# Westlake-AI/SemiReward

Hardware: AMD Instinct MI355X
Metric: unlabeled images/sec/node (FlexMatch+SR, ViT-S CIFAR-100) (higher is better)
Workload: dtype bf16

## Files before the change

### semireward_amd/csrc/attn_block.hip

```cpp
#include <stdlib.h>

#include <type_traits>
#include <utility>

#include "../../include/srhip.h"
#include "common.h"

namespace {

constexpr int HD = 64;
constexpr int DM = 384;
constexpr int NH = DM / HD;
constexpr int KS = DM / 32;
constexpr int SK = 64;
constexpr int ST_EL = 64 * SK;
constexpr int NS = 8;
constexpr int GS = 2;
constexpr int NG = NS / GS;
constexpr int SPM = DM / SK;
constexpr int SPH = 3 * SPM;
constexpr int NSTG = NH * SPH;
constexpr float LOG2E = 1.4426950408889634f;

typedef __attribute__((address_space(3))) void lds_void;
template <int N_>
__device__ __forceinline__ void wait_vm() { asm volatile("s_waitcnt vmcnt(%0)" ::"n"(N_) : "memory"); }
__device__ __forceinline__ void lds_barrier() {
  asm volatile("s_waitcnt lgkmcnt(0)" ::: "memory");
  __builtin_amdgcn_s_barrier();
  asm volatile("" ::: "memory");
}

__device__ __forceinline__ int fresh_lane() {
  int l;
  asm volatile("v_mbcnt_lo_u32_b32 %0, -1, 0\n\tv_mbcnt_hi_u32_b32 %0, -1, %0" : "=v"(l));
  return l;
}

__device__ __forceinline__ float max3_raw(float a, float b, float c) {
  return __builtin_amdgcn_fmed3f(__builtin_amdgcn_fmed3f(a, b, INFINITY), c, INFINITY);
}
__device__ __forceinline__ float rows_max(float x) {
  const unsigned u = __float_as_uint(x);
  const auto a = __builtin_amdgcn_permlane16_swap(u, u, false, false);
  const unsigned v = __float_as_uint(__builtin_amdgcn_fmed3f(__uint_as_float(a[0]), __uint_as_float(a[1]), INFINITY));
  const auto b = __builtin_amdgcn_permlane32_swap(v, v, false, false);
  return __builtin_amdgcn_fmed3f(__uint_as_float(b[0]), __uint_as_float(b[1]), INFINITY);
}
__device__ __forceinline__ float rows_sum(float x) {
  const unsigned u = __float_as_uint(x);
  const auto a = __builtin_amdgcn_permlane16_swap(u, u, false, false);
  const unsigned v = __float_as_uint(__uint_as_float(a[0]) + __uint_as_float(a[1]));
  const auto b = __builtin_amdgcn_permlane32_swap(v, v, false, false);
  return __uint_as_float(b[0]) + __uint_as_float(b[1]);
}

__device__ __forceinline__ f32x4_t mfma16(u32x4_t a, u32x4_t b, f32x4_t c) {
  return __builtin_amdgcn_mfma_f32_16x16x32_bf16(__builtin_bit_cast(bf16x8_t, a), __builtin_bit_cast(bf16x8_t, b), c, 0, 0, 0);
}
__device__ __forceinline__ u32x4_t ldf(const bf16_t* p) { return *reinterpret_cast<const u32x4_t*>(p); }
__device__ __forceinline__ u32x4_t pack8v(f32x4_t lo, f32x4_t hi) {
  return u32x4_t{pack_bf2(lo[0], lo[1]), pack_bf2(lo[2], lo[3]), pack_bf2(hi[0], hi[1]), pack_bf2(hi[2], hi[3])};
}
constexpr int vt_pitch(int NP) { return ((NP / 2) % 64 == 16 || (NP / 2) % 64 == 48) ? NP : NP + 32; }
__device__ __forceinline__ int swz4(int row) { return (0x78 >> (((row >> 2) & 3) * 2)) & 3; }
constexpr int nkt_of(int N) { return 2 * ((N + 31) / 32); }

template <class F, int... Is>
__device__ __forceinline__ void static_for_impl(F&& f, std::integer_sequence<int, Is...>) { (f(std::integral_constant<int, Is>{}), ...); }
template <int N, class F>
__device__ __forceinline__ void static_for(F&& f) { static_for_impl(f, std::make_integer_sequence<int, N>{}); }

struct AbArgs {
  const bf16_t* xnb;
  const bf16_t* qx;
  const float* bqkv;
  const bf16_t* W;
  bf16_t* out;
  const float* osc;
  float scale;
  int B;
};

template <int N, int DBG>
__global__ __launch_bounds__(512, 2) void attn_block_kernel(AbArgs a) {
  constexpr int NKT = nkt_of(N), NP = NKT * 16, TP = vt_pitch(NP);
  constexpr int NQT = (N + 15) / 16;
  constexpr bool EXTRA = NQT == 17;
  static_assert(NQT <= 16 || (EXTRA && N == 257), "two token tiles per wave (+ one extra token)");
  constexpr int NKT_LO = (N - 1) / 16;
  extern __shared__ __attribute__((aligned(16))) bf16_t sm[];
  bf16_t* ring = sm;
  bf16_t* Ks = ring + NS * ST_EL;
  bf16_t* Vt = Ks + NP * HD;
  bf16_t* sx = Vt + HD * TP;
  float* sbias = reinterpret_cast<float*>(sx + 3 * DM);
  const int tid = threadIdx.x, lane = tid & 63;
  const int wave = __builtin_amdgcn_readfirstlane(tid >> 6);
  const int l15 = lane & 15, g = lane >> 4;
  const int img = blockIdx.x;
  const float osc = a.osc ? a.osc[img] : 1.0f;
  const int hpw = NH / gridDim.y, hbeg = blockIdx.y * hpw, hend = hbeg + hpw;
  const size_t row0 = (size_t)img * N;

  const int rho = 8 * wave + (lane >> 3);
  const int srcc = (lane & 7) ^ ((rho >> 1) & 7);
  const int fperm = (rho & 32) + 8 * ((rho & 15) >> 2) + 4 * ((rho >> 4) & 1) + (rho & 3);
  const int vo_kq = (fperm * DM + srcc * 8) * 2, vo_v = (rho * DM + srcc * 8) * 2;
  const __amdgpu_buffer_rsrc_t rw = __builtin_amdgcn_make_buffer_rsrc(const_cast<bf16_t*>(a.W), 0, 3 * DM * DM * 2, 0x00020000);
  constexpr int OOB = 0x7ffffff0;
  auto issue = [&](auto rc, int h) __attribute__((always_inline)) {
    constexpr int r0 = decltype(rc)::value, r = r0 % SPH, m = r / SPM, kc = r % SPM;
    const int hh = h + r0 / SPH;
    const bool valid = hh < hend;
    constexpr int brow = m == 0 ? DM : m == 1 ? 2 * DM : 0;
    lds_void* dst = (lds_void*)(ring + (r0 % NS >= 0 ? ((hh * SPH + r) & (NS - 1)) : 0) * ST_EL + wave * 8 * SK);
    if constexpr ((DBG & 4) != 0) return;
    __builtin_amdgcn_raw_ptr_buffer_load_lds(rw, dst, 16, valid ? (m == 1 ? vo_v : vo_kq) : OOB,
                                             valid ? ((brow + hh * HD) * DM + kc * SK) * 2 : 0, 0, 0);
  };
  issue(std::integral_constant<int, 0>{}, hbeg); issue(std::integral_constant<int, 1>{}, hbeg);
  issue(std::integral_constant<int, 2>{}, hbeg); issue(std::integral_constant<int, 3>{}, hbeg);
  static_assert((NG - 2) * GS == 4, "prologue issues the first two groups");

  for (int i = tid; i < 3 * DM; i += 512) sbias[i] = a.bqkv[i];
  if (EXTRA && tid < 3 * DM / 8) reinterpret_cast<u32x4_t*>(sx)[tid] = ldf(a.qx + (size_t)img * 3 * DM + 8 * tid);
  for (int i = tid; i < (NP - N) * HD / 8; i += 512) reinterpret_cast<u32x4_t*>(Ks + N * HD)[i] = u32x4_t{0u, 0u, 0u, 0u};
  for (int i = tid; i < HD * TP / 8; i += 512) reinterpret_cast<u32x4_t*>(Vt)[i] = u32x4_t{0u, 0u, 0u, 0u};
  __syncthreads();

  u32x4_t xn[2][KS];
#pragma unroll
  for (int tt = 0; tt < 2; ++tt) {
    const bool have = tt == 0 || NQT - (EXTRA ? 1 : 0) == 16 || wave + 8 < NQT - (EXTRA ? 1 : 0);
    const int tok = min(16 * (wave + 8 * tt) + l15, N - 1);
    const bf16_t* xr = a.xnb + (row0 + tok) * DM + 8 * g;
#pragma unroll
    for (int k = 0; k < KS; ++k) xn[tt][k] = have ? ldf(xr + 32 * k) : u32x4_t{0u, 0u, 0u, 0u};
  }

  const int kc_ = g ^ ((l15 >> 1) & 7);
  const int fo0 = l15 * SK + (kc_ << 3), fo1 = l15 * SK + ((kc_ ^ 4) << 3);
  const int kof0 = l15 * HD + (kc_ << 3), kof1 = l15 * HD + ((kc_ ^ 4) << 3);
  const int vof = l15 * TP + ((g ^ swz4(l15)) << 3);
  const float sc2 = a.scale * LOG2E;

  auto sync_group = [&](auto rc, int h) __attribute__((always_inline)) {
    constexpr int r = decltype(rc)::value;
    if constexpr ((DBG & 4) == 0) wait_vm<GS*(NG - 3)>();
    __builtin_amdgcn_s_barrier();
    if constexpr ((DBG & 32) == 0) {
      issue(std::integral_constant<int, r + (NG - 2) * GS>{}, h);
      issue(std::integral_constant<int, r + (NG - 2) * GS + 1>{}, h);
    }
    static_assert(GS == 2, "two stages per group");
  };
  constexpr bool ALL2 = NQT - (EXTRA ? 1 : 0) == 16;
  const bool tile1 = ALL2 || wave + 8 < NQT - (EXTRA ? 1 : 0);

  u32x4_t qf[2][2];
  auto project = [&](auto mc, int h) __attribute__((always_inline)) {
    constexpr int M = decltype(mc)::value;
    f32x4_t acc[2][4];
    const float* bb = sbias + (M == 0 ? DM : M == 1 ? 2 * DM : 0) + h * HD;
#pragma unroll
    for (int t = 0; t < 4; ++t) {
      f32x4_t b4;
      if constexpr (M == 1) { const float b = bb[16 * t + l15]; b4 = f32x4_t{b, b, b, b}; }
      else b4 = *reinterpret_cast<const f32x4_t*>(bb + 32 * (t >> 1) + 8 * g + 4 * (t & 1));
      acc[0][t] = b4; acc[1][t] = b4;
    }
    u32x4_t fa[2][2];
    auto rd = [&](auto uc) __attribute__((always_inline)) {
      constexpr int u = decltype(uc)::value, j = u >> 1, hf = u & 1, stg = j >> 1, sh = j & 1;
      const bf16_t* tile = ring + ((h * SPH + M * SPM + stg) & (NS - 1)) * ST_EL;
      fa[u & 1][0] = ldf(tile + (2 * hf) * 16 * SK + (sh ? fo1 : fo0));
      fa[u & 1][1] = ldf(tile + (2 * hf + 1) * 16 * SK + (sh ? fo1 : fo0));
    };
    auto mm = [&](auto uc) __attribute__((always_inline)) {
      constexpr int u = decltype(uc)::value, j = u >> 1, hf = u & 1;
      u32x4_t(&fr)[2] = fa[u & 1];
      if constexpr ((DBG & 2) != 0) {
        asm volatile("" ::"v"(fr[0]), "v"(fr[1]));
      } else if constexpr (M != 1) {
#pragma unroll
        for (int t = 0; t < 2; ++t) {
          acc[0][2 * hf + t] = mfma16(fr[t], xn[0][j], acc[0][2 * hf + t]);
          acc[1][2 * hf + t] = mfma16(fr[t], xn[1][j], acc[1][2 * hf + t]);
        }
      } else {
#pragma unroll
        for (int t = 0; t < 2; ++t) {
          acc[0][2 * hf + t] = mfma16(xn[0][j], fr[t], acc[0][2 * hf + t]);
          acc[1][2 * hf + t] = mfma16(xn[1][j], fr[t], acc[1][2 * hf + t]);
        }
      }
    };
    sync_group(std::integral_constant<int, M * SPM>{}, h);
    rd(std::integral_constant<int, 0>{});
    static_for<2 * KS>([&](auto uc) __attribute__((always_inline)) {
      constexpr int u = decltype(uc)::value;
      if constexpr (u + 1 < 2 * KS) {
        if constexpr ((u + 1) % (4 * GS) == 0) sync_group(std::integral_constant<int, M * SPM + (u + 1) / 4>{}, h);
        rd(std::integral_constant<int, u + 1>{});
      }
      __builtin_amdgcn_sched_barrier(0);
      mm(uc);
      __builtin_amdgcn_sched_barrier(0);
      if constexpr ((DBG & 32) != 0 && u % 4 == 0) issue(std::integral_constant<int, M * SPM + u / 4 + (NG - 2) * GS>{}, h);
    });
    if constexpr (M == 0) {
      const int lnk = fresh_lane(), l15k = lnk & 15, gk = lnk >> 4;
#pragma unroll
      for (int tt = 0; tt < 2; ++tt) {
        if (tt == 1 && !tile1) break;
        const int key = 16 * (wave + 8 * tt) + l15k;
#pragma unroll
        for (int blk = 0; blk < 2; ++blk)
          *reinterpret_cast<u32x4_t*>(Ks + key * HD + (((4 * blk + gk) ^ ((key >> 1) & 7)) << 3)) = pack8v(acc[tt][2 * blk], acc[tt][2 * blk + 1]);
      }
      if (EXTRA && wave == 0) {
        const int ln_ = fresh_lane();
        if (ln_ < 8) *reinterpret_cast<u32x4_t*>(Ks + 256 * HD + (ln_ << 3)) = ldf(sx + DM + h * HD + 8 * ln_);
      }
    } else if constexpr (M == 1) {
      const int lnv = fresh_lane(), l15v = lnv & 15, gv = lnv >> 4;
#pragma unroll
      for (int tt = 0; tt < 2; ++tt) {
        if (tt == 1 && !tile1) break;
        const int T = wave + 8 * tt, u = T >> 1, e = T & 1;
#pragma unroll
        for (int t = 0; t < 4; ++t) {
          const int d = 16 * t + l15v;
          *reinterpret_cast<u32x2_t*>(Vt + d * TP + 32 * u + ((gv ^ swz4(d)) << 3) + 4 * e) =
              u32x2_t{pack_bf2(acc[tt][t][0], acc[tt][t][1]), pack_bf2(acc[tt][t][2], acc[tt][t][3])};
        }
      }
      if (EXTRA && wave == 1) {
        const int ln_ = fresh_lane();
        Vt[ln_ * TP + 256 + (swz4(ln_) << 3)] = sx[2 * DM + h * HD + ln_];
      }
    } else {
#pragma unroll
      for (int tt = 0; tt < 2; ++tt) {
        qf[tt][0] = pack8v(acc[tt][0], acc[tt][1]);
        qf[tt][1] = pack8v(acc[tt][2], acc[tt][3]);
      }
    }
  };
  using C0 = std::integral_constant<int, 0>;
  using C1 = std::integral_constant<int, 1>;
  using C2 = std::integral_constant<int, 2>;

#pragma unroll 1
  for (int h = hbeg; h < hend; ++h) {
    project(C0{}, h);
    project(C1{}, h);
    project(C2{}, h);
    lds_barrier();

    const int nq = (DBG & 1) ? 0 : (tile1 ? 2 : 1) + ((EXTRA && (DBG & 8) == 0 && (h & 7) == wave) ? 1 : 0);
#pragma unroll 1
    for (int qi = 0; qi < nq; ++qi) {
      const bool ext = EXTRA && qi == (tile1 ? 2 : 1);
      int qtok;
      if (ext) { qf[0][0] = ldf(sx + h * HD + 8 * g); qf[0][1] = ldf(sx + h * HD + 32 + 8 * g); qtok = 256 + l15; }
      else qtok = 16 * (wave + 8 * qi) + l15;
      const u32x4_t q0 = qf[0][0], q1 = qf[0][1];
      constexpr int CHT = 4, NCH = (NKT + CHT - 1) / CHT;
      f32x4_t o[4];
#pragma unroll
      for (int dt = 0; dt < 4; ++dt) o[dt] = f32x4_t{0.f, 0.f, 0.f, 0.f};
      float mrun = -INFINITY;
      f32x2_t psum = {0.f, 0.f};
      static_for<NCH>([&](auto cc) __attribute__((always_inline)) {
        constexpr int ch = decltype(cc)::value, t0 = ch * CHT, nt = (NKT - t0 < CHT) ? NKT - t0 : CHT;
        static_assert(nt % 2 == 0, "the PV product consumes key-tile pairs");
        f32x4_t s[nt];
        float mx = -INFINITY;
#pragma unroll
        for (int i = 0; i < nt; ++i) {
          const int t = t0 + i;
          const int nvalid = N - 16 * t;
          if (nvalid <= 0) continue;
          f32x4_t c = {0.f, 0.f, 0.f, 0.f};
          c = mfma16(ldf(Ks + t * 16 * HD + kof0), q0, c);
          c = mfma16(ldf(Ks + t * 16 * HD + kof1), q1, c);
          if (nvalid >= 16) {
            mx = max3_raw(mx, c[0], c[1]);
            mx = max3_raw(mx, c[2], c[3]);
          } else {
#pragma unroll
            for (int r = 0; r < 4; ++r) {
              if (r < nvalid) { c[r] = (4 * g + r < nvalid) ? c[r] : -INFINITY; mx = max3_raw(mx, c[r], c[r]); }
            }
          }
          s[i] = c;
          if ((i & 1) == 1) __builtin_amdgcn_sched_barrier(0);
        }
        mx = rows_max(mx);
        const float mnew = max3_raw(mrun, mx, mx);
        const float nmx = -mnew * sc2;
        if constexpr (ch > 0) {
          const float corr = fast_exp2(fmaf(mrun, sc2, nmx));
          psum *= corr;
#pragma unroll
          for (int dt = 0; dt < 4; ++dt) o[dt] *= corr;
        }
        mrun = mnew;
        const f32x4_t sc4 = {sc2, sc2, sc2, sc2}, nm4 = {nmx, nmx, nmx, nmx};
#pragma unroll
        for (int i = 0; i < nt; ++i) {
          const int nvalid = N - 16 * (t0 + i);
          if (nvalid >= 16) {
            const f32x4_t e = __builtin_elementwise_fma(s[i], sc4, nm4);
            const f32x4_t p = (DBG & 16) ? e : f32x4_t{fast_exp2(e[0]), fast_exp2(e[1]), fast_exp2(e[2]), fast_exp2(e[3])};
            s[i] = p;
            psum += f32x2_t{p[0], p[1]};
            psum += f32x2_t{p[2], p[3]};
          } else {
            f32x4_t p = {0.f, 0.f, 0.f, 0.f};
#pragma unroll
            for (int r = 0; r < 4; ++r)
              if (r < nvalid) { p[r] = fast_exp2(fmaf(s[i][r], sc2, nmx)); psum[r & 1] += p[r]; }
            s[i] = p;
          }
        }
#pragma unroll
        for (int u = 0; u < nt / 2; ++u) {
          const u32x4_t pb = pack8v(s[2 * u], s[2 * u + 1]);
#pragma unroll
          for (int dt = 0; dt < 4; ++dt) o[dt] = mfma16(ldf(Vt + dt * 16 * TP + 32 * (t0 / 2 + u) + vof), pb, o[dt]);
          __builtin_amdgcn_sched_barrier(0);
        }
      });
      float sum = psum[0] + psum[1];
      sum = rows_sum(sum);
      if (qtok < N && (!ext || l15 == 0)) {
        const float inv = osc / sum;
        bf16_t* op = a.out + (row0 + qtok) * DM + h * HD + g * 4;
#pragma unroll
        for (int dt = 0; dt < 4; ++dt) {
          uint2 v = {pack_bf2(o[dt][0] * inv, o[dt][1] * inv), pack_bf2(o[dt][2] * inv, o[dt][3] * inv)};
          *reinterpret_cast<uint2*>(op + dt * 16) = v;
        }
      }
      qf[0][0] = qf[1][0]; qf[0][1] = qf[1][1];
    }
  }
}

template <int N, int DBG = 0>
int launch(const AbArgs& a, hipStream_t s) {
  constexpr int NKT = nkt_of(N), NP = NKT * 16, TP = vt_pitch(NP);
  const size_t smem = (size_t)(NS * ST_EL + NP * HD + HD * TP + 3 * DM) * sizeof(bf16_t) + (size_t)(3 * DM) * sizeof(float);
  auto kern = attn_block_kernel<N, DBG>;
  (void)hipFuncSetAttribute((const void*)kern, hipFuncAttributeMaxDynamicSharedMemorySize, (int)smem);
  int split = 1;
  for (int c : {2, 3, 6}) if (a.B * c <= 256) split = c;
  if (const char* e = SR_TUNE_ENV("SRHIP_AB_SPLIT")) { const int v = atoi(e); if (v == 1 || v == 2 || v == 3 || v == 6) split = v; }
  SR_LAUNCH(kern, dim3(a.B, split), dim3(512), smem, s, a);
  SR_CHECK_LAUNCH();
  return SR_OK;
}

}

extern "C" int srhip_attn_block_supported(int N, int D, int H) { return (D == DM && H == NH && (N == 257 || N == 197)) ? 1 : 0; }

extern "C" int srhip_attn_block_fused(const void* xn_bf16, const void* Wqkv, const float* bqkv, const void* qkv_extra, void* out,
                                      const float* out_scale, int B, int N, int D, int H, float scale, void* stream) {
  if (!xn_bf16 || !Wqkv || !bqkv || !out || B <= 0) return SR_EINVAL;
  if (!srhip_attn_block_supported(N, D, H)) return SR_EINVAL;
  if (N == 257 && !qkv_extra) return SR_EINVAL;
  if (((uintptr_t)xn_bf16 | (uintptr_t)Wqkv | (uintptr_t)out | (uintptr_t)bqkv | (uintptr_t)qkv_extra) & 15) return SR_EINVAL;
  AbArgs a;
  a.xnb = (const bf16_t*)xn_bf16; a.qx = (const bf16_t*)qkv_extra; a.bqkv = bqkv; a.W = (const bf16_t*)Wqkv; a.out = (bf16_t*)out;
  a.scale = scale; a.B = B; a.osc = out_scale;
  hipStream_t s = (hipStream_t)stream;
#ifdef SRHIP_TUNING
  switch (SR_TUNE_ENV("SRHIP_AB_DEBUG") ? atoi(SR_TUNE_ENV("SRHIP_AB_DEBUG")) : 0) {
    case 1: return N == 257 ? launch<257, 1>(a, s) : launch<197, 1>(a, s);
    case 2: return N == 257 ? launch<257, 2>(a, s) : launch<197, 2>(a, s);
    case 3: return N == 257 ? launch<257, 3>(a, s) : launch<197, 3>(a, s);
    case 4: return N == 257 ? launch<257, 4>(a, s) : launch<197, 4>(a, s);
    case 6: return N == 257 ? launch<257, 6>(a, s) : launch<197, 6>(a, s);
    case 7: return N == 257 ? launch<257, 7>(a, s) : launch<197, 7>(a, s);
    case 8: return N == 257 ? launch<257, 8>(a, s) : launch<197, 8>(a, s);
    case 16: return N == 257 ? launch<257, 16>(a, s) : launch<197, 16>(a, s);
    default: break;
  }
#endif
  static const int spread = SR_TUNE_ENV("SRHIP_ATTN_SPREAD") ? atoi(SR_TUNE_ENV("SRHIP_ATTN_SPREAD")) : 1;
  if (spread) return N == 257 ? launch<257, 32>(a, s) : launch<197, 32>(a, s);
  return N == 257 ? launch<257>(a, s) : launch<197>(a, s);
}
```

### semireward_amd/ops.py

```python
import ctypes
import os

import torch

from . import _lib
from ._lib import EPI_BF16, EPI_DGELU_BF16, EPI_F32, EPI_GELU_BF16, EPI_RESID_F32
from ._lib import X3_EPI_F32, X3_EPI_GELU_F32, X3_EPI_RESID_F32
from ._lib import X3B_NT, X3B_NN, X3B_EPI_F32, X3B_EPI_ACC, X3B_EPI_DGELU, X3B_EPI_GELU_PRE
from ._lib import REDUCE_NONE, REDUCE_MEAN, REDUCE_SUM


_CHECK_ARGS = os.environ.get("SRHIP_CHECK_ARGS", "0") != "0"


def _p_checked(t):
    if t is None:
        return None
    assert t.is_cuda and t.is_contiguous(), "libsrhip needs contiguous device tensors"
    return t.data_ptr()


def _p_fast(t):
    return None if t is None else t.data_ptr()

# ... 246 lines not shown
        if n > self.bufs[slot].numel():
            return torch.from_numpy(arr_u8.copy()).to(device)
        if self.events[slot] is not None:
            self.events[slot].synchronize()
        self.bufs[slot][:n].copy_(torch.from_numpy(arr_u8))
        dev = torch.empty(n, dtype=torch.uint8, device=device)
        dev.copy_(self.bufs[slot][:n], non_blocking=True)
        ev = torch.cuda.Event()
        ev.record()
        self.events[slot] = ev
        return dev


SLAB_DESC_DTYPE = [("dst", "<u8"), ("src", "<u8"), ("stride", "<i8"), ("count", "<i4"), ("n_slabs", "<i4"), ("block_start", "<i4"), ("pad0", "<i4")]
TN_OVERWRITE = 2


def make_group_tn_desc(problems, device, split_k=0, tile=128, slabs=False, stager=None):
    import numpy as np
    assert all(pr[6] > 0 and pr[4] % 8 == 0 and pr[5] % 8 == 0 for pr in problems), "K >= 1 tokens; M, N multiples of 8 (srhip.h)"
    plan = [(tuple(pr), split_k if (split_k > 0 and pr[6] >= 2 * split_k) else 0) for pr in problems]
    if tile == 256 and split_k == 0:
        plan = tn_pp_plan(problems)
    slabs = slabs and any(sk > 0 for _, sk in plan)
    lay, n_el = [], 0
    if slabs:
        for (A, B, C, db, M, N, K), sk in plan:
            if sk > 0:
                nsl = -(-K // sk)
                oc = n_el
                n_el += nsl * M * N
                ob = n_el
                n_el += nsl * M if db is not None else 0
                n_el = -(-n_el // 4) * 4
                lay.append((oc, ob, nsl))
            else:
                lay.append(None)
        slab = torch.empty(max(n_el, 4), dtype=torch.float32, device=device)
    ent, red = [], []
    t = rb = 0
    for i, ((A, B, C, db, M, N, K), sk) in enumerate(plan):
        tiles = ((M + tile - 1) // tile) * ((N + tile - 1) // tile)
        if sk > 0:
            for si, k0 in enumerate(range(0, K, sk)):
                if slabs:
                    oc, ob, nsl = lay[i]
                    cp = slab.data_ptr() + 4 * (oc + si * M * N)
                    bp = slab.data_ptr() + 4 * (ob + si * M) if db is not None else 0
                    ent.append((_p(A) + 2 * k0 * M, _p(B) + 2 * k0 * N, cp, bp, M, N, min(sk, K - k0), M, N, N, t, TN_OVERWRITE))
                else:
                    ent.append((_p(A) + 2 * k0 * M, _p(B) + 2 * k0 * N, _p(C), _p(db) or 0, M, N, min(sk, K - k0), M, N, N, t, TN_ATOMIC))
                t += tiles
            if slabs:
                oc, ob, nsl = lay[i]
                red.append((_p(C), slab.data_ptr() + 4 * oc, M * N, M * N, nsl, rb, 0))
                rb += -(-M * N // 1024)
                if db is not None:
                    red.append((_p(db), slab.data_ptr() + 4 * ob, M, M, nsl, rb, 0))
                    rb += -(-M // 1024)
        else:
            ent.append((_p(A), _p(B), _p(C), _p(db) or 0, M, N, K, M, N, N, t, 0))
            t += tiles
    arr = np.zeros(len(ent), dtype=GROUP_TN_DESC_DTYPE)
    for i, e in enumerate(ent):
        arr[i] = e
    assert arr.itemsize == 64
    flops = float(sum(2.0 * M * N * K for *_, M, N, K in problems))
    nbytes = float(sum(2.0 * (M * K + N * K) + 8.0 * M * N for *_, M, N, K in problems))
    up = (lambda a: stager.upload(a.view(np.uint8).reshape(-1), device)) if stager is not None else (lambda a: torch.from_numpy(a.view(np.uint8).copy()).to(device))
    desc = up(arr)
    desc.out_ranges = [(e[2], 4 * e[4] * e[5]) for e in ent] + [(e[3], 4 * e[4]) for e in ent if e[3]]
    if slabs:
        ra = np.zeros(len(red), dtype=SLAB_DESC_DTYPE)
        for i, e in enumerate(red):
            ra[i] = e
        assert ra.itemsize == 40
        desc.slab = slab
        desc.reduce = (up(ra), len(red), rb)
    return desc, len(ent), t, flops, nbytes


TN_PP_GRID = 256


def tn_pp_plan(problems, grid=TN_PP_GRID):
    tiles = [((M + 255) // 256) * ((N + 255) // 256) for *_, M, N, K in problems]
    total = sum(tiles)
    rem = total % grid
    plan = [(tuple(pr), 0) for pr in problems]
    if total < grid or rem == 0 or rem > 0.7 * grid:
        return plan
    got = 0
    for i in range(len(problems) - 1, -1, -1):
        if got >= rem:
            break
        K = problems[i][6]
        want = max(2, min(8, grid // max(rem, 1)))
        n = min(want, K // 512)
        if n >= 2:
            sl = -(-K // n)
            sl = -(-sl // 64) * 64
            plan[i] = (tuple(problems[i]), sl)
        got += tiles[i]
    return plan


def tn_pp_efficiency(problems):
    area = sum(M * N for *_, M, N, K in problems)
    cover = sum(((M + 255) // 256) * ((N + 255) // 256) * 65536 for *_, M, N, K in problems)
    return area / max(cover, 1)


def gemm_tn_grouped_f32(desc, n_problems, total_tiles, alpha=1.0, beta=1.0, flops=0.0, nbytes=0.0, pp=False):
    fn, kern = ("srhip_gemm_tn_grouped_pp_f32", "gemm_tn_pp_kernel") if pp else ("srhip_gemm_tn_grouped_f32", "gemm_tn_grouped_f32_kernel")
    red = getattr(desc, "reduce", None)
    if red is not None:
        assert beta == 1.0, "a table with slab slices is a C += product"
    if _PROFILE is not None:
        _PROFILE.timed(fn, (_p(desc), n_problems, total_tiles, alpha, beta, _s(),), flops, kern, nbytes)
    else:
        _call(fn, _p(desc), n_problems, total_tiles, alpha, beta, _s())
    if red is not None:
        _call("srhip_slab_reduce_f32", _p(red[0]), red[1], red[2], _s())


def gemm_tn_grouped_tail_f32(desc, n_problems, total_tiles, D, ln=None, head=None, pe=None, alpha=1.0, beta=1.0):
    from ._lib import DwTail
    assert getattr(desc, "reduce", None) is None, "a table with slab slices has a second phase of its own"
    t = DwTail()
    t.D = D
    if ln is not None:
        t.ln_desc, t.ln_part, t.n_ln, t.n_rep = _p(ln[0]), _p(ln[1]), ln[2], ln[3]
    if head is not None:
        t.dlogits, t.feat, t.dWh, t.dbh, t.B, t.C = _p(head[0]), _p(head[1]), _p(head[2]), _p(head[3]), head[4], head[5]
    if pe is not None:
        assert head is None or head[4] == pe[6]
        t.dx, t.img, t.img_index, t.dpos, t.dcls, t.pe_ws = (_p(x) for x in pe[:6])
        t.B, t.in_chans, t.HW, t.ps = pe[6:]
    if _CHECK_ARGS:
        mine = list(getattr(ln[0], "out_ranges", ())) if ln is not None else []
        mine += [(_p(x), x.numel() * x.element_size()) for x in ((head[2], head[3]) if head is not None else ()) + (tuple(pe[3:6]) if pe is not None else ())]
        for a0, an in mine:
            for b0, bn in getattr(desc, "out_ranges", ()):
                assert a0 + an <= b0 or b0 + bn <= a0, "a tail output of gemm_tn_grouped_tail_f32 overlaps a C / dbias of the table"
    _call("srhip_gemm_tn_grouped_tail_f32", _p(desc), n_problems, total_tiles, alpha, beta, ctypes.addressof(t), _s())


def attn_block_supported(N, D, H):
    from ._lib import lib
    return bool(lib().srhip_attn_block_supported(N, D, H))


def attn_block_fused(xn, Wqkv, bqkv, out, B, N, D, H, scale, qkv_extra=None, out_scale=None):
    if N == 257:
        gemm_nt(EPI_BF16, xn[256:], Wqkv, qkv_extra, B, 3 * D, D, lda=N * D, bias=bqkv)
    if _PROFILE is not None:
        M = B * N
        _PROFILE.timed("srhip_attn_block_fused", (_p(xn), _p(Wqkv), _p(bqkv), _p(qkv_extra), _p(out), _p(out_scale), B, N, D, H, scale, _s(),), 2.0 * M * 3 * D * D + 4.0 * B * H * N * N * 64, "attn_block_kernel<%d>" % N,
                              2.0 * M * D + 2.0 * M * D + 2.0 * 3 * D * D)
        return
    _call("srhip_attn_block_fused", _p(xn), _p(Wqkv), _p(bqkv), _p(qkv_extra), _p(out), _p(out_scale), B, N, D, H, scale, _s())


def attn_fwd(qkv, out, lse, B, N, H, scale):
    if _PROFILE is not None:
        _PROFILE.timed("srhip_attn_fwd", (_p(qkv), _p(out), _p(lse), B, N, H, scale, _s()), 4.0 * B * H * N * N * 64, "attn_fwd_kernel",
                       2.0 * B * N * 4 * H * 64)
        return
    _call("srhip_attn_fwd", _p(qkv), _p(out), _p(lse), B, N, H, scale, _s())


def attn_bwd(qkv, out, d_out, lse, dqkv, delta_ws, B, N, H, scale):
    if _PROFILE is not None:
        _PROFILE.timed("srhip_attn_bwd", (_p(qkv), _p(out), _p(d_out), _p(lse), _p(dqkv), _p(delta_ws), B, N, H, scale, _s()),
                       10.0 * B * H * N * N * 64, "attn_bwd (dq + dkv kernels)", 2.0 * B * N * 8 * H * 64)
        return
    _call("srhip_attn_bwd", _p(qkv), _p(out), _p(d_out), _p(lse), _p(dqkv), _p(delta_ws), B, N, H, scale, _s())


def layernorm_fwd(x, gamma, beta, eps, out, mean, rstd, M, D):
    _call("srhip_layernorm_fwd", _p(x), _p(gamma), _p(beta), eps, _p(out), _p(mean), _p(rstd), M, D, _s())


def layernorm_bwd_cast(dy, x, mean, rstd, gamma, dx, dgamma, dbeta, out_bf16, row_scale, rows_per_sample, M, D):
    _call("srhip_layernorm_bwd_cast", _p(dy), _p(x), _p(mean), _p(rstd), _p(gamma), _p(dx), _p(dgamma), _p(dbeta), _p(out_bf16), _p(row_scale),
          rows_per_sample, M, D, _s())


def layernorm_bwd_part(dy, x, mean, rstd, gamma, dx, part, n_rep, out_bf16, row_scale, rows_per_sample, M, D):
    if _PROFILE is not None:
        _PROFILE.timed("srhip_layernorm_bwd_part", (_p(dy), _p(x), _p(mean), _p(rstd), _p(gamma), _p(dx), _p(part), n_rep, _p(out_bf16),
                                                    _p(row_scale), rows_per_sample, M, D, _s()), 0.0, "ln_bwd_kernel", 16.0 * M * D)
        return
    _call("srhip_layernorm_bwd_part", _p(dy), _p(x), _p(mean), _p(rstd), _p(gamma), _p(dx), _p(part), n_rep, _p(out_bf16), _p(row_scale),
          rows_per_sample, M, D, _s())


def make_ln_reduce_desc(pairs, device):
    import numpy as np
    arr = np.array([[_p(g), _p(b)] for g, b in pairs], dtype=np.uint64)
    desc = torch.from_numpy(arr.view(np.uint8).copy()).to(device)
    desc.out_ranges = [(_p(t), t.numel() * t.element_size()) for pair in pairs for t in pair]
    return desc


def ln_grad_reduce(desc, part, n_ln, n_rep, D):
    _call("srhip_ln_grad_reduce", _p(desc), _p(part), n_ln, n_rep, D, _s())


def mlp_fused(x, gamma, beta, eps, W1, b1, W2, b2, row_scale, rows_per_sample, M, D, Hd, x_out=None, save=None):
    rows, ln2, pre, h, mean, rstd = save if save is not None else (0, None, None, None, None, None)
    args = (_p(x), _p(x_out if x_out is not None else x), _p(gamma), _p(beta), eps, _p(W1), _p(b1), _p(W2), _p(b2), _p(row_scale),
            rows_per_sample, rows, _p(ln2), _p(pre), _p(h), _p(mean), _p(rstd), M, D, Hd)
    if _PROFILE is not None:
        _PROFILE.timed("srhip_mlp_fused", (*args, _s(),), 4.0 * M * D * Hd, "mlp_fused_kernel<384, 0, 4>",
                              8.0 * M * D + 4.0 * D * Hd + rows * (2.0 * D + 4.0 * Hd))
        return
    _call("srhip_mlp_fused", *args, _s())


def mlp_fused_proj(x, ao, Wp, bp, row_scale1, gamma, beta, eps, W1, b1, W2, b2, row_scale2, rows_per_sample, M, D, Hd, x_out=None,
                   ln_next=None, next_gamma=None, next_beta=None, ao_scaled=False):
    args = (_p(x), _p(x_out if x_out is not None else x), _p(ao), _p(Wp), _p(bp), _p(row_scale1), int(bool(ao_scaled)), _p(gamma), _p(beta), eps,
            _p(W1), _p(b1),
            _p(W2), _p(b2), _p(row_scale2), rows_per_sample, _p(ln_next), _p(next_gamma), _p(next_beta), M, D, Hd)
    if _PROFILE is not None:
        _PROFILE.timed("srhip_mlp_fused_proj", (*args, _s(),), 4.0 * M * D * Hd + 2.0 * M * D * D, "mlp_fused_kernel<384, 0, 4, true, 1>",
                              8.0 * M * D + 2.0 * M * D + (2.0 * M * D if ln_next is not None else 0.0) + 4.0 * D * Hd + 2.0 * D * D)
        return
    _call("srhip_mlp_fused_proj", *args, _s())


def gelu_eval(x, y_erf, y_poly):
    _call("srhip_gelu_eval", _p(x), _p(y_erf), _p(y_poly), x.numel(), _s())


def layernorm_bwd(dy, x, mean, rstd, gamma, dx, dgamma, dbeta, M, D):
    _call("srhip_layernorm_bwd", _p(dy), _p(x), _p(mean), _p(rstd), _p(gamma), _p(dx), _p(dgamma), _p(dbeta), M, D, _s())


def patch_embed_fwd(img, img_index, Wp, bp, cls, pos, x, B, C, HW, ps, D):
    _call("srhip_patch_embed_fwd", _p(img), _p(img_index), _p(Wp), _p(bp), _p(cls), _p(pos), _p(x), B, C, HW, ps, D, _s())


def patch_embed_bwd(dx, img, img_index, dWp, dbp, dcls, dpos, B, C, HW, ps, D):
    _call("srhip_patch_embed_bwd", _p(dx), _p(img), _p(img_index), _p(dWp), _p(dbp), _p(dcls), _p(dpos), B, C, HW, ps, D, _s())


def patch_embed_bwd_ws_floats(B, C, HW, ps, D):
    n = int(_lib.lib().srhip_patch_embed_bwd_ws_floats(B, C, HW, ps, D))
    if n < 0:
        raise ValueError("srhip_patch_embed_bwd_ws refuses B=%d C=%d HW=%d ps=%d D=%d" % (B, C, HW, ps, D))
    return n


def patch_embed_bwd_ws(dx, img, img_index, dWp, dbp, dcls, dpos, ws, B, C, HW, ps, D, part_done=False):
    if part_done:
        _call("srhip_patch_embed_bwd_fold", _p(ws), _p(dWp), _p(dbp), B, C, HW, ps, D, _s())
        return
    _call("srhip_patch_embed_bwd_ws", _p(dx), _p(img), _p(img_index), _p(dWp), _p(dbp), _p(dcls), _p(dpos), _p(ws), B, C, HW, ps, D, _s())


def patch_im2col(img, img_index, out, B, C, HW, ps):
    _call("srhip_patch_im2col", _p(img), _p(img_index), _p(out), B, C, HW, ps, _s())


def patch_assemble(tok, bp, cls, pos, x, B, Np, D):
    _call("srhip_patch_assemble", _p(tok), _p(bp), _p(cls), _p(pos), _p(x), B, Np, D, _s())


def patch_grad_operands(dx, dx_tok, dpos, dcls, B, Np, D):
    _call("srhip_patch_grad_operands", _p(dx), _p(dx_tok), _p(dpos), _p(dcls), B, Np, D, _s())


def gemm_nt_x3(epi, A, W, C, M, N, K, *, lda=None, ldw=None, ldc=None, bias=None, row_scale=None, rows_per_sample=0):
    args = (epi, _p(A), lda or K, _p(W), ldw or K, _p(C), ldc or N, M, N, K, _p(bias), _p(row_scale), rows_per_sample, _s())
    if _PROFILE is not None:
        _PROFILE.timed("srhip_gemm_nt_x3", args, 2.0 * M * N * K, "gemm_nt_x3_kernel<%d>" % epi,
                       4.0 * (M * K + N * K) + 4.0 * M * N * (2 if epi == X3_EPI_RESID_F32 else 1))
        return
    _call("srhip_gemm_nt_x3", *args)


def attn_fwd_x3(qkv, out, B, N, H, scale):
    if _PROFILE is not None:
        _PROFILE.timed("srhip_attn_fwd_x3", (_p(qkv), _p(out), B, N, H, scale, _s()), 4.0 * B * H * N * N * 64, "attn_fwd_x3_kernel",
                       4.0 * B * N * 4 * H * 64)
        return
    _call("srhip_attn_fwd_x3", _p(qkv), _p(out), B, N, H, scale, _s())


def layernorm_fwd_f32(x, gamma, beta, eps, out, mean, rstd, M, D):
    _call("srhip_layernorm_fwd_f32", _p(x), _p(gamma), _p(beta), eps, _p(out), _p(mean), _p(rstd), M, D, _s())


def patch_im2col_f32(img, img_index, out, B, C, HW, ps):
    _call("srhip_patch_im2col_f32", _p(img), _p(img_index), _p(out), B, C, HW, ps, _s())


def attn_fwd_x3_lse(qkv, out, lse, B, N, H, scale):
    args = (_p(qkv), _p(out), _p(lse), B, N, H, scale, _s())
    if _PROFILE is not None:
        _PROFILE.timed("srhip_attn_fwd_x3_lse", args, 4.0 * B * H * N * N * 64, "attn_fwd_x3_lse_kernel", 4.0 * B * N * 4 * H * 64)
        return
    _call("srhip_attn_fwd_x3_lse", *args)


def gemm_x3(layout, epi, A, B, C, M, N, K, *, lda=None, ldb=None, ldc=None, bias=None, aux=None, aux_out=None, ldaux=0):
# ... 679 lines not shown
```

Measured before the change: 1674.

## Fuse extra-token QKV projection into attention block kernel, drop separate GEMM

For N=257, the 257th token's Q/K/V projection was computed by a separate gemm_nt launch before the fused attention kernel. That projection now runs inside the kernel. Waves do extra MFMAs against the weight tiles already staged in the LDS ring, reduce partial sums through a small shared buffer and write the result into Ks, Vt and a Q slot. This removes a kernel launch and a global round trip, at the cost of extra LDS traffic, registers and MFMA work in the projection loop. It also switches K/V fragment loads to explicit LDS address-space pointers.

```diff
diff --git a/semireward_amd/csrc/attn_block.hip b/semireward_amd/csrc/attn_block.hip
--- a/semireward_amd/csrc/attn_block.hip
+++ b/semireward_amd/csrc/attn_block.hip
@@ -23,6 +23,12 @@
 constexpr float LOG2E = 1.4426950408889634f;
 
 typedef __attribute__((address_space(3))) void lds_void;
+typedef __attribute__((address_space(3))) u32x4_t lds_u32x4;
+__device__ __forceinline__ const lds_u32x4* lds_base(const bf16_t* p) {
+  const lds_u32x4* q = (const lds_u32x4*)p;
+  asm volatile("" : "+v"(q));
+  return q;
+}
 template <int N_>
 __device__ __forceinline__ void wait_vm() { asm volatile("s_waitcnt vmcnt(%0)" ::"n"(N_) : "memory"); }
 __device__ __forceinline__ void lds_barrier() {
@@ -65,6 +71,8 @@
 constexpr int vt_pitch(int NP) { return ((NP / 2) % 64 == 16 || (NP / 2) % 64 == 48) ? NP : NP + 32; }
 __device__ __forceinline__ int swz4(int row) { return (0x78 >> (((row >> 2) & 3) * 2)) & 3; }
 constexpr int nkt_of(int N) { return 2 * ((N + 31) / 32); }
+constexpr int sx_elems(int N) { return N == 257 ? DM + HD : 3 * DM; }
+constexpr int part_elems(int N) { return N == 257 ? 4 * HD : 0; }
 
 template <class F, int... Is>
 __device__ __forceinline__ void static_for_impl(F&& f, std::integer_sequence<int, Is...>) { (f(std::integral_constant<int, Is>{}), ...); }
@@ -73,7 +81,6 @@
 
 struct AbArgs {
   const bf16_t* xnb;
-  const bf16_t* qx;
   const float* bqkv;
   const bf16_t* W;
   bf16_t* out;
@@ -93,8 +100,10 @@
   bf16_t* ring = sm;
   bf16_t* Ks = ring + NS * ST_EL;
   bf16_t* Vt = Ks + NP * HD;
-  bf16_t* sx = Vt + HD * TP;
-  float* sbias = reinterpret_cast<float*>(sx + 3 * DM);
+  bf16_t* sxn = Vt + HD * TP;
+  bf16_t* sxq = sxn + DM;
+  float* sbias = reinterpret_cast<float*>(sxn + sx_elems(N));
+  float* part = sbias + 3 * DM;
   const int tid = threadIdx.x, lane = tid & 63;
   const int wave = __builtin_amdgcn_readfirstlane(tid >> 6);
   const int l15 = lane & 15, g = lane >> 4;
@@ -124,7 +133,7 @@
   static_assert((NG - 2) * GS == 4, "prologue issues the first two groups");
 
   for (int i = tid; i < 3 * DM; i += 512) sbias[i] = a.bqkv[i];
-  if (EXTRA && tid < 3 * DM / 8) reinterpret_cast<u32x4_t*>(sx)[tid] = ldf(a.qx + (size_t)img * 3 * DM + 8 * tid);
+  if (EXTRA && tid < DM / 8) reinterpret_cast<u32x4_t*>(sxn)[tid] = ldf(a.xnb + (row0 + 256) * DM + 8 * tid);
   for (int i = tid; i < (NP - N) * HD / 8; i += 512) reinterpret_cast<u32x4_t*>(Ks + N * HD)[i] = u32x4_t{0u, 0u, 0u, 0u};
   for (int i = tid; i < HD * TP / 8; i += 512) reinterpret_cast<u32x4_t*>(Vt)[i] = u32x4_t{0u, 0u, 0u, 0u};
   __syncthreads();
@@ -143,6 +152,16 @@
   const int fo0 = l15 * SK + (kc_ << 3), fo1 = l15 * SK + ((kc_ ^ 4) << 3);
   const int kof0 = l15 * HD + (kc_ << 3), kof1 = l15 * HD + ((kc_ ^ 4) << 3);
   const int vof = l15 * TP + ((g ^ swz4(l15)) << 3);
+  const lds_u32x4 *kb0 = nullptr, *kb1 = nullptr, *vb = nullptr;
+  if constexpr (EXTRA) { kb0 = lds_base(Ks + kof0); kb1 = lds_base(Ks + kof1); vb = lds_base(Vt + vof); }
+  auto ldk = [&](int t, int half) __attribute__((always_inline)) {
+    if constexpr (EXTRA) return (half ? kb1 : kb0)[t * 16 * HD / 8];
+    else return ldf(Ks + t * 16 * HD + (half ? kof1 : kof0));
+  };
+  auto ldv = [&](int dt, int kp) __attribute__((always_inline)) {
+    if constexpr (EXTRA) return vb[(dt * 16 * TP + 32 * kp) / 8];
+    else return ldf(Vt + dt * 16 * TP + 32 * kp + vof);
+  };
   const float sc2 = a.scale * LOG2E;
 
   auto sync_group = [&](auto rc, int h) __attribute__((always_inline)) {
@@ -158,6 +177,27 @@
   constexpr bool ALL2 = NQT - (EXTRA ? 1 : 0) == 16;
   const bool tile1 = ALL2 || wave + 8 < NQT - (EXTRA ? 1 : 0);
 
+  float pr[5];
+  auto extra_reduce_load = [&](auto mp, int h) __attribute__((always_inline)) {
+    constexpr int MP = decltype(mp)::value;
+    if (MP == 2 || wave == MP) {
+      const int f = fresh_lane();
+#pragma unroll
+      for (int w = 0; w < 4; ++w) pr[w] = part[w * HD + f];
+      pr[4] = sbias[(MP == 0 ? DM : MP == 1 ? 2 * DM : 0) + h * HD + f];
+    }
+  };
+  auto extra_reduce_store = [&](auto mp) __attribute__((always_inline)) {
+    constexpr int MP = decltype(mp)::value;
+    if (MP == 2 || wave == MP) {
+      const int f = fresh_lane();
+      const float s = (((pr[0] + pr[1]) + pr[2]) + pr[3]) + pr[4];
+      if constexpr (MP == 0) Ks[256 * HD + f] = f2bf(s);
+      else if constexpr (MP == 1) Vt[f * TP + 256 + (swz4(f) << 3)] = f2bf(s);
+      else sxq[f] = f2bf(s);
+    }
+  };
+
   u32x4_t qf[2][2];
   auto project = [&](auto mc, int h) __attribute__((always_inline)) {
     constexpr int M = decltype(mc)::value;
@@ -171,6 +211,26 @@
       acc[0][t] = b4; acc[1][t] = b4;
     }
     u32x4_t fa[2][2];
+    u32x4_t xe, fe[2];
+    const lds_u32x4 *xb = nullptr, *fb = nullptr;
+    f32x4_t xa[2];
+    if constexpr (EXTRA) {
+      const int lne = fresh_lane(), l15e = lne & 15, ge = lne >> 4;
+      xb = lds_base(sxn + 32 * (wave & 3) + 8 * ge);
+      fb = lds_base(ring + (32 * (wave >> 2) + l15e) * SK + (((ge ^ ((l15e >> 1) & 7)) ^ ((wave & 1) << 2)) << 3));
+      xa[0] = f32x4_t{0.f, 0.f, 0.f, 0.f}; xa[1] = f32x4_t{0.f, 0.f, 0.f, 0.f};
+    }
+    auto rd_extra = [&](auto gc) __attribute__((always_inline)) {
+      constexpr int gi = decltype(gc)::value;
+      const int slot = (h * SPH + M * SPM + GS * gi + ((wave >> 1) & 1)) & (NS - 1);
+      xe = xb[(4 * gi) * 32 / 8];
+      fe[0] = fb[slot * (ST_EL / 8)];
+      fe[1] = fb[slot * (ST_EL / 8) + 16 * SK / 8];
+    };
+    auto mm_extra = [&]() __attribute__((always_inline)) {
+#pragma unroll
+      for (int t = 0; t < 2; ++t) xa[t] = M != 1 ? mfma16(fe[t], xe, xa[t]) : mfma16(xe, fe[t], xa[t]);
+    };
     auto rd = [&](auto uc) __attribute__((always_inline)) {
       constexpr int u = decltype(uc)::value, j = u >> 1, hf = u & 1, stg = j >> 1, sh = j & 1;
       const bf16_t* tile = ring + ((h * SPH + M * SPM + stg) & (NS - 1)) * ST_EL;
@@ -198,17 +258,34 @@
     };
     sync_group(std::integral_constant<int, M * SPM>{}, h);
     rd(std::integral_constant<int, 0>{});
+    if constexpr (EXTRA && M != 0) extra_reduce_load(std::integral_constant<int, M - 1>{}, h);
     static_for<2 * KS>([&](auto uc) __attribute__((always_inline)) {
       constexpr int u = decltype(uc)::value;
+      if constexpr (EXTRA && u % (4 * GS) == 0) rd_extra(std::integral_constant<int, u / (4 * GS)>{});
       if constexpr (u + 1 < 2 * KS) {
         if constexpr ((u + 1) % (4 * GS) == 0) sync_group(std::integral_constant<int, M * SPM + (u + 1) / 4>{}, h);
         rd(std::integral_constant<int, u + 1>{});
       }
       __builtin_amdgcn_sched_barrier(0);
       mm(uc);
+      if constexpr (EXTRA && u % (4 * GS) == 2) mm_extra();
       __builtin_amdgcn_sched_barrier(0);
+      if constexpr (EXTRA && M != 0 && u == 1) extra_reduce_store(std::integral_constant<int, M - 1>{});
       if constexpr ((DBG & 32) != 0 && u % 4 == 0) issue(std::integral_constant<int, M * SPM + u / 4 + (NG - 2) * GS>{}, h);
     });
+    if constexpr (EXTRA) {
+      const int lnx = fresh_lane(), l15x = lnx & 15, gx = lnx >> 4;
+      float* pw = part + (wave & 3) * HD + 32 * (wave >> 2);
+      if constexpr (M == 1) {
+        if (gx == 0) { pw[l15x] = xa[0][0]; pw[16 + l15x] = xa[1][0]; }
+      } else {
+        if (l15x == 0) {
+          *reinterpret_cast<f32x4_t*>(pw + 8 * gx) = xa[0];
+          *reinterpret_cast<f32x4_t*>(pw + 8 * gx + 4) = xa[1];
+        }
+      }
+      asm volatile("s_waitcnt lgkmcnt(0)" ::: "memory");
+    }
     if constexpr (M == 0) {
       const int lnk = fresh_lane(), l15k = lnk & 15, gk = lnk >> 4;
 #pragma unroll
@@ -218,10 +295,6 @@
 #pragma unroll
         for (int blk = 0; blk < 2; ++blk)
           *reinterpret_cast<u32x4_t*>(Ks + key * HD + (((4 * blk + gk) ^ ((key >> 1) & 7)) << 3)) = pack8v(acc[tt][2 * blk], acc[tt][2 * blk + 1]);
-      }
-      if (EXTRA && wave == 0) {
-        const int ln_ = fresh_lane();
-        if (ln_ < 8) *reinterpret_cast<u32x4_t*>(Ks + 256 * HD + (ln_ << 3)) = ldf(sx + DM + h * HD + 8 * ln_);
       }
     } else if constexpr (M == 1) {
       const int lnv = fresh_lane(), l15v = lnv & 15, gv = lnv >> 4;
@@ -235,10 +308,6 @@
           *reinterpret_cast<u32x2_t*>(Vt + d * TP + 32 * u + ((gv ^ swz4(d)) << 3) + 4 * e) =
               u32x2_t{pack_bf2(acc[tt][t][0], acc[tt][t][1]), pack_bf2(acc[tt][t][2], acc[tt][t][3])};
         }
-      }
-      if (EXTRA && wave == 1) {
-        const int ln_ = fresh_lane();
-        Vt[ln_ * TP + 256 + (swz4(ln_) << 3)] = sx[2 * DM + h * HD + ln_];
       }
     } else {
 #pragma unroll
@@ -264,7 +333,11 @@
     for (int qi = 0; qi < nq; ++qi) {
       const bool ext = EXTRA && qi == (tile1 ? 2 : 1);
       int qtok;
-      if (ext) { qf[0][0] = ldf(sx + h * HD + 8 * g); qf[0][1] = ldf(sx + h * HD + 32 + 8 * g); qtok = 256 + l15; }
+      if (ext) {
+        extra_reduce_load(std::integral_constant<int, 2>{}, h);
+        extra_reduce_store(std::integral_constant<int, 2>{});
+        qf[0][0] = ldf(sxq + 8 * g); qf[0][1] = ldf(sxq + 32 + 8 * g); qtok = 256 + l15;
+      }
       else qtok = 16 * (wave + 8 * qi) + l15;
       const u32x4_t q0 = qf[0][0], q1 = qf[0][1];
       constexpr int CHT = 4, NCH = (NKT + CHT - 1) / CHT;
@@ -284,8 +357,8 @@
           const int nvalid = N - 16 * t;
           if (nvalid <= 0) continue;
           f32x4_t c = {0.f, 0.f, 0.f, 0.f};
-          c = mfma16(ldf(Ks + t * 16 * HD + kof0), q0, c);
-          c = mfma16(ldf(Ks + t * 16 * HD + kof1), q1, c);
+          c = mfma16(ldk(t, 0), q0, c);
+          c = mfma16(ldk(t, 1), q1, c);
           if (nvalid >= 16) {
             mx = max3_raw(mx, c[0], c[1]);
             mx = max3_raw(mx, c[2], c[3]);
@@ -330,7 +403,7 @@
         for (int u = 0; u < nt / 2; ++u) {
           const u32x4_t pb = pack8v(s[2 * u], s[2 * u + 1]);
 #pragma unroll
-          for (int dt = 0; dt < 4; ++dt) o[dt] = mfma16(ldf(Vt + dt * 16 * TP + 32 * (t0 / 2 + u) + vof), pb, o[dt]);
+          for (int dt = 0; dt < 4; ++dt) o[dt] = mfma16(ldv(dt, t0 / 2 + u), pb, o[dt]);
           __builtin_amdgcn_sched_barrier(0);
         }
       });
@@ -353,7 +426,7 @@
 template <int N, int DBG = 0>
 int launch(const AbArgs& a, hipStream_t s) {
   constexpr int NKT = nkt_of(N), NP = NKT * 16, TP = vt_pitch(NP);
-  const size_t smem = (size_t)(NS * ST_EL + NP * HD + HD * TP + 3 * DM) * sizeof(bf16_t) + (size_t)(3 * DM) * sizeof(float);
+  const size_t smem = (size_t)(NS * ST_EL + NP * HD + HD * TP + sx_elems(N)) * sizeof(bf16_t) + (size_t)(3 * DM + part_elems(N)) * sizeof(float);
   auto kern = attn_block_kernel<N, DBG>;
   (void)hipFuncSetAttribute((const void*)kern, hipFuncAttributeMaxDynamicSharedMemorySize, (int)smem);
   int split = 1;
@@ -375,7 +448,7 @@
   if (N == 257 && !qkv_extra) return SR_EINVAL;
   if (((uintptr_t)xn_bf16 | (uintptr_t)Wqkv | (uintptr_t)out | (uintptr_t)bqkv | (uintptr_t)qkv_extra) & 15) return SR_EINVAL;
   AbArgs a;
-  a.xnb = (const bf16_t*)xn_bf16; a.qx = (const bf16_t*)qkv_extra; a.bqkv = bqkv; a.W = (const bf16_t*)Wqkv; a.out = (bf16_t*)out;
+  a.xnb = (const bf16_t*)xn_bf16; a.bqkv = bqkv; a.W = (const bf16_t*)Wqkv; a.out = (bf16_t*)out;
   a.scale = scale; a.B = B; a.osc = out_scale;
   hipStream_t s = (hipStream_t)stream;
 #ifdef SRHIP_TUNING
diff --git a/semireward_amd/ops.py b/semireward_amd/ops.py
--- a/semireward_amd/ops.py
+++ b/semireward_amd/ops.py
@@ -422,8 +422,6 @@
 
 
 def attn_block_fused(xn, Wqkv, bqkv, out, B, N, D, H, scale, qkv_extra=None, out_scale=None):
-    if N == 257:
-        gemm_nt(EPI_BF16, xn[256:], Wqkv, qkv_extra, B, 3 * D, D, lda=N * D, bias=bqkv)
     if _PROFILE is not None:
         M = B * N
         _PROFILE.timed("srhip_attn_block_fused", (_p(xn), _p(Wqkv), _p(bqkv), _p(qkv_extra), _p(out), _p(out_scale), B, N, D, H, scale, _s(),), 2.0 * M * 3 * D * D + 4.0 * B * H * N * N * 64, "attn_block_kernel<%d>" % N,
```

Result: no change. 1677 (median of 4 runs) (+0.2%).
